# GetOverMassif/QSP-SLAM

Hardware: AMD Instinct MI355X
Metric: joint-opt iters/sec (BA+SDF) (higher is better)
Workload: dtype f32 as 2 x fp16 per operand (hi + 2^-11 lo'), 3 fp16 products per multiply-add, f32 accumulate (decoder); f64 (bundle adjustment)

## Files before the change

### include/qsp_hip.h

```cpp
#ifndef QSP_HIP_H
#define QSP_HIP_H

#include <stddef.h>
#include <stdint.h>

#ifdef __cplusplus
extern "C" {
#endif

enum {
    QSP_OK = 0,
    QSP_ERR_INVALID = 1,
    QSP_ERR_UNSUPPORTED = 2,
    QSP_ERR_DEVICE = 3,
    QSP_ERR_NO_DEVICE = 4
};

const char* qsp_last_error(void);
int qsp_version(void);
int qsp_device_count(void);


typedef struct {
    int32_t n_layers;
    int32_t code_len;
    int32_t latent_in_layer;
    const int32_t* in_dim;
    const int32_t* out_dim;
    const float* const* weight;
    const float* const* weight_g;
    const float* const* bias;
} qsp_decoder_desc;

typedef struct qsp_decoder qsp_decoder;

int qsp_decoder_create(const qsp_decoder_desc* desc, int device, qsp_decoder** out);
void qsp_decoder_destroy(qsp_decoder* dec);

enum { QSP_DEC_OPT_FORWARD_PRECISION = 1, QSP_DEC_OPT_JACOBIAN_PRECISION = 2, QSP_DEC_OPT_TILE_POINTS = 3,
       QSP_DEC_OPT_RENDER_SCREENING = 4, QSP_DEC_OPT_USE_TANH = 5, QSP_DEC_OPT_RANGE_FALLBACK = 6,
       QSP_DEC_OPT_SCREENING_MIN_SAMPLES = 7, QSP_DEC_OPT_NARROW_TILE = 8, QSP_DEC_OPT_SCREEN_AUDIT = 9,
       QSP_DEC_OPT_DEPTH_STAGING = 10 };
enum { QSP_DEC_CNT_RANGE_FALLBACKS = 1, QSP_DEC_CNT_ARENA_REUSED = 2, QSP_DEC_CNT_ARENA_CREATED = 3, QSP_DEC_CNT_NARROW_TILE = 4,
       QSP_DEC_CNT_SCREEN_FALLBACKS = 5 };
int64_t qsp_decoder_get_counter(qsp_decoder* dec, int32_t counter);
int qsp_decoder_set_option(qsp_decoder* dec, int32_t option, int32_t value);

int qsp_decode_sdf(qsp_decoder* dec, const float* code, const float* xyz, int64_t n, float* sdf_out);

int qsp_decode_sdf_screen(qsp_decoder* dec, const float* code, const float* xyz, int64_t n, float* s1_out);

int qsp_sdf_value_grad(qsp_decoder* dec, const float* code, const float* xyz, int64_t n, float* y, float* grad);

typedef struct {
    float k1, k2, k3, k4;
    float b1, b2;
    float lr;
    float s_damp;
    float cut_off;
    int32_t n_iter;
    int32_t n_depth;
    int32_t code_len;
} qsp_joint_cfg;

typedef struct qsp_refine_batch qsp_refine_batch;

int qsp_refine_batch_create(qsp_decoder* dec, const qsp_joint_cfg* cfg, int32_t n_obj,
                            const float* const* pts, const int32_t* n_pts,
                            const float* const* rays, const int32_t* n_rays,
                            const float* const* depth, const int32_t* n_fg,
                            int32_t n_hyp, const int32_t* hyp_obj, qsp_refine_batch** out);
void qsp_refine_batch_destroy(qsp_refine_batch* b);

int qsp_refine_batch_set_state(qsp_refine_batch* b, const float* t_cam_obj, const float* code);

// ... 518 lines not shown
```

### qsp_slam_amd/csrc/sdf_kernels.hpp

```cpp
#pragma once
#include <hip/hip_runtime.h>
#include <math.h>
#include <stdint.h>

#include "common.hpp"
#include "sdf_mlp.hpp"

namespace qsp {

constexpr int MAX_DEPTH = 64;
#ifndef QSP_NW_REND
#define QSP_NW_REND 16
#endif
#ifndef QSP_NW_SDF_MAX
#define QSP_NW_SDF_MAX 256
#endif
constexpr int NW_REND = QSP_NW_REND;
constexpr int NW_SDF_MAX = QSP_NW_SDF_MAX;
constexpr int NH = 71;
constexpr int PART_FLOATS = ((NJ * (NJ + 1) / 2 + 31) / 32) * 32;
__device__ __forceinline__ int tri72(int r, int c) { return r * NJ - (r * (r - 1)) / 2 + (c - r); }
__device__ __forceinline__ void part_store(float* __restrict__ slot, int ta, int tb, int lane, const f32x16& hacc) {
    const int r0 = 32 * ta + 4 * (lane >> 5), c = 32 * tb + (lane & 31);
    const int k = (NJ - 1) - r0, m = c < NJ ? c - r0 : -1;
// ... 565 lines not shown
        }
    }
    if (band_idx && screen_dmax && threadIdx.x < 64) {
#pragma unroll
        for (int o = 32; o > 0; o >>= 1) dmax = fmaxf(dmax, __shfl_xor(dmax, o, 64));
        if (threadIdx.x == 0 && dmax > 0.f) atomicMax(screen_dmax, __float_as_uint(dmax));
    }
    if (!(amax <= H2_MAX)) *P->range_flag = 1;
}

template <int NW, bool GRP = false>
__global__ __launch_bounds__(64 * NW) void k_mlp_fwd_h1(HypState* __restrict__ st, const ObjView* __restrict__ objs,
                                                            const float* __restrict__ rays, RefineCfg cfg, const MlpParams* __restrict__ P,
                                                            const int32_t* __restrict__ valid_rk, int64_t rk_stride,
                                                            float* __restrict__ sdf_valid, const int2* __restrict__ work,
                                                            int* __restrict__ qctl, const float* __restrict__ c0_all,
                                                            int32_t* __restrict__ band_idx, float band_th, int audit_one_in,
                                                            const int32_t* __restrict__ stage_idx) {
    extern __shared__ __attribute__((aligned(16))) unsigned char smem_raw[];
    MlpSmemH1& s = *reinterpret_cast<MlpSmemH1*>(smem_raw);
    __shared__ float Tsh[16];
    __shared__ int s_item;
    const int n_items = qctl[0];
    float amax = 0.f;
    int h_cached = -1;
    [[maybe_unused]] int dec_staged = -1;
    if constexpr (!GRP) {
        const MlpParams& Pp = *P;
        for (int i = threadIdx.x; i < HID; i += 64 * NW) s.w8[i] = Pp.w8[i];
#pragma unroll
        for (int l = 1; l < 8; ++l)
            for (int i = threadIdx.x; i < HID; i += 64 * NW) s.bias[(l - 1) * HID + i] = Pp.bias[l][i];
    }
    for (;;) {
        if (threadIdx.x == 0) s_item = atomicAdd(&qctl[1], 1);
        __syncthreads();
        const int item = s_item;
        if (item >= n_items) break;
        const int h = work[item].x, t = work[item].y;
        HypState& S = st[h];
        const int n = stage_idx ? S.n_stage : S.n_valid;
        const int32_t* stg = stage_idx ? stage_idx + h * rk_stride : nullptr;
        const ObjView ov = objs[S.obj];
        const float* R = rays + 3 * ov.ray_off;
        const int32_t* rk = valid_rk + h * rk_stride;
        float* out = sdf_valid + h * rk_stride;
        if (h != h_cached) {
            if (threadIdx.x >= 64 && threadIdx.x < 80) Tsh[threadIdx.x - 64] = S.T_oc[threadIdx.x - 64];
            for (int i = threadIdx.x; i < HID; i += 64 * NW) {
                s.c0[i] = c0_all[(size_t)h * 2 * HID + i];
                s.c4[i] = c0_all[(size_t)h * 2 * HID + HID + i];
            }
            h_cached = h;
        }
        if constexpr (GRP) {
            if (ov.dec != dec_staged) {
                const MlpParams& Pp = P[ov.dec];
                for (int i = threadIdx.x; i < HID; i += 64 * NW) s.w8[i] = Pp.w8[i];
#pragma unroll
                for (int l = 1; l < 8; ++l)
                    for (int i = threadIdx.x; i < HID; i += 64 * NW) s.bias[(l - 1) * HID + i] = Pp.bias[l][i];
                dec_staged = ov.dec;
            }
        }
        const float d_min = S.d_min, d_max = S.d_max;
        __syncthreads();
        if (threadIdx.x < H1_ROWS) {
            const int v = t * H1_ROWS + threadIdx.x;
            float x = 0, y = 0, z = 0;
            if (v < n) {
                const int e = rk[stg ? stg[v] : v];
                const int r = e >> 6, k = e & 63;
                const float d = depth_at(d_min, d_max, k, cfg.n_depth);
                xform(Tsh, R[3 * r] * d, R[3 * r + 1] * d, R[3 * r + 2] * d, x, y, z);
            }
            s.xin[4 * threadIdx.x + 0] = x;
            s.xin[4 * threadIdx.x + 1] = y;
            s.xin[4 * threadIdx.x + 2] = z;
            s.xin[4 * threadIdx.x + 3] = 0.f;
        }
        __syncthreads();
        if constexpr (GRP) mlp_tile_h1<2, NW>(s, P + ov.dec, amax);
        else mlp_tile_h1<2, NW>(s, P, amax);
        if (threadIdx.x < H1_ROWS) {
            int v = t * H1_ROWS + threadIdx.x;
            bool in = false, audit = false;
            if (v < n) {
                if (stg) v = stg[v];
                const float y = s.y[threadIdx.x];
                out[v] = y;
                in = !(fabsf(y) >= band_th);
                audit = !in && screen_audit_pick(h, v, cfg.iter, audit_one_in);
            }
            const unsigned long long m = __ballot(in || audit);
            const int lane = threadIdx.x & 63;
            int base = 0;
            if (lane == 0 && m) base = atomicAdd(&S.n_band, __popcll(m));
            base = __builtin_amdgcn_readfirstlane(base);
            if (in || audit) band_idx[h * rk_stride + base + __popcll(m & ((1ull << lane) - 1ull))] = audit ? (v | BAND_AUDIT_BIT) : v;
        }
    }
    if (!(amax <= H2_MAX)) *P->range_flag = 1;
}

struct RayScan {
    float d_u;
    int n_emit;
};

constexpr float SCAN_NONE = 1e30f;
constexpr int SCAN_RAYS = 512;
constexpr int SCAN_LD = MAX_DEPTH + 1;
__device__ __forceinline__ int scan_ray(float* row, int D, float d_min, float d_max, float th, float depth_obs, uint64_t& kept,
                                        float& res_out) {
    float occ[MAX_DEPTH];
    float Tl[MAX_DEPTH];
    uint64_t inband = 0;
    float acc = 1.f, d_u = 0.f;
#pragma unroll
    for (int k = 0; k < MAX_DEPTH; ++k) {
        if (k < D) {
            const float s = row[k];
            float o = 0.f;
            if (s < 0.5f * SCAN_NONE) {
                const float c = fminf(fmaxf(s, -th), th);
                o = 0.5f - c / (2.f * th);
                if (s > -th && s < th) inband |= 1ull << k;
            }
            occ[k] = o;
            const float d = depth_at(d_min, d_max, k, D);
            d_u += d * (o * acc);
            acc *= (1.f - o);
            Tl[k] = acc;
// ... 235 lines not shown
#pragma unroll 8
            for (int ks = 0; ks < TILE_P / 2; ++ks) hacc = mfma32t<!B3>(A[2 * ks * LDJ], B[2 * ks * LDJ], hacc);
            mfma_acc_settle<!B3>(hacc);
        }
        QSP_TSK(4)
    }
    if (wave < 6) part_store(partials + ((int64_t)h * nw_total + slot) * PART_FLOATS, ta, tb, lane, hacc);
    QSP_TSK(5)
    tsk_first = false;
  }
}

struct JtjArgs {
    const HypState* st;
    const ObjView* objs;
    const float* pts;
    const float* rays;
    RefineCfg cfg;
    const MlpParams* P;
    int nw_sdf, nw_total;
    const int32_t* rend_rk;
    const float* rend_deds;
    const float* rend_res;
    int64_t rk_stride;
    const uint8_t* pt_active;
    int64_t act_stride;
    float* res_out;
    float* rows_out;
    int64_t rows_stride;
    float* partials;
    const int2* work;
    int* qctl;
    const float* c0_all;
};
typedef const __attribute__((address_space(4))) JtjArgs* jtj_kargs_t;
__device__ __forceinline__ jtj_kargs_t jtj_kernargs() {
    auto p = __builtin_amdgcn_kernarg_segment_ptr();
    asm volatile("" : "+s"(p));
    return (jtj_kargs_t)p;
}

template <int NR, int NW = 4, bool NARROW = false, bool GRP = false>
__global__ __launch_bounds__(64 * NW) void k_mlp_jtj_h2(JtjArgs ) {
    constexpr int NT = 64 * NW;
    extern __shared__ __attribute__((aligned(16))) unsigned char smem_raw[];
    MlpSmem& s = *reinterpret_cast<MlpSmem*>(smem_raw);
    __shared__ float Tsh[16];
    __shared__ int s_item;
    constexpr int TP = 32 * NR, SUBS = NT / TP;
    [[maybe_unused]] bool staged = false;
    float amax = 0.f;
    int item = -1, t = 0;
    [[maybe_unused]] int dec = 0, dec_staged = -1;
    for (;;) {
        {
            const jtj_kargs_t A = jtj_kernargs();
            int tid = threadIdx.x;
            asm volatile("" : "+v"(tid));
            const bool fresh = item < 0;
            if (fresh) {
                if (tid == 0) s_item = atomicAdd(&A->qctl[3], 1);
                __syncthreads();
                item = __builtin_amdgcn_readfirstlane(s_item);
                if (item >= A->qctl[2]) break;
            } else {
                __syncthreads();
            }
            const int2 wk = A->work[item];
            const int h = wk.x, slot = wk.y;
            const HypState& S = A->st[h];
            const ObjView ov = A->objs[S.obj];
            const int nw_sdf = A->nw_sdf;
            const bool is_sdf = slot < nw_sdf;
            const int n = is_sdf ? ov.n_pts : S.n_render;
            if constexpr (GRP) dec = __builtin_amdgcn_readfirstlane(ov.dec);
            if (fresh) {
                t = is_sdf ? slot : slot - nw_sdf;
                if (tid < CODE_LEN) s.code[tid] = S.code[tid];
                if (tid >= 64 && tid < 80) Tsh[tid - 64] = S.T_oc[tid - 64];
                const float* c0 = A->c0_all + (size_t)h * 2 * HID;
                for (int i = tid; i < HID; i += NT) {
                    s.c0[i] = c0[i];
                    s.c4[i] = c0[HID + i];
                }
                __syncthreads();
            }
            if (tid < TP) {
                const int v = t * TP + tid;
                float x = 0, y = 0, z = 0, sc = 0.f, rr = 0.f;
                if (v < n) {
                    if (is_sdf) {
                        const float* Pc = A->pts + 3 * ov.pts_off;
                        const uint8_t* active = A->pt_active ? A->pt_active + h * A->act_stride : nullptr;
                        xform(Tsh, Pc[3 * v], Pc[3 * v + 1], Pc[3 * v + 2], x, y, z);
                        sc = (active && !active[v]) ? 0.f : 1.f;
                    } else {
                        const float* R = A->rays + 3 * ov.ray_off;
                        const int64_t ro = h * A->rk_stride;
                        const int e = A->rend_rk[ro + v];
                        const int r = e >> 6, k = e & 63;
                        const float d = depth_at(S.d_min, S.d_max, k, A->cfg.n_depth);
                        xform(Tsh, R[3 * r] * d, R[3 * r + 1] * d, R[3 * r + 2] * d, x, y, z);
                        sc = A->rend_deds[ro + v];
                        rr = A->rend_res[ro + v];
                    }
                }
                s.xin[4 * tid + 0] = x;
                s.xin[4 * tid + 1] = y;
                s.xin[4 * tid + 2] = z;
                s.xin[4 * tid + 3] = (v < n) ? 1.f : 0.f;
                s.rscale[tid] = sc;
                s.rres[tid] = rr;
            }
            __syncthreads();
        }
        {
            if constexpr (GRP) {
                const MlpParams* Pm = jtj_kernargs()->P + dec;
                mlp_tile_h2<true, 2, false, NR, NW, NARROW>(s, Pm, amax, dec != dec_staged);
                dec_staged = dec;
            } else {
                const MlpParams* Pm = jtj_kernargs()->P;
                mlp_tile_h2<true, 2, false, NR, NW, NARROW>(s, Pm, amax, !staged);
                staged = true;
            }
        }
        {
            asm volatile("" : "+s"(item), "+s"(t));
            const jtj_kargs_t A = jtj_kernargs();
            int tid = threadIdx.x;
            asm volatile("" : "+v"(tid));
            const int wave = __builtin_amdgcn_readfirstlane(tid >> 6), lane = tid & 63;
            const int2 wk = A->work[item];
            const int h = wk.x, slot = wk.y;
            const HypState& S = A->st[h];
            const ObjView ov = A->objs[S.obj];
            const int nw_sdf = A->nw_sdf, nw_total = A->nw_total;
            const bool is_sdf = slot < nw_sdf;
            const int n = is_sdf ? ov.n_pts : S.n_render;
            const int j0 = is_sdf ? slot : slot - nw_sdf;
            const int stride = is_sdf ? nw_sdf : nw_total - nw_sdf;
            const int pose_only = A->cfg.pose_only;
            const float hub = is_sdf ? A->cfg.b2 : A->cfg.b1;
            float* G = s.act;
            float* Jt = s.act + TILE_P * LDG;
            {
                const int p = tid / SUBS, sub = tid % SUBS;
                const float valid = s.xin[4 * p + 3];
                const float sc = s.rscale[p] * valid;
#pragma unroll
                for (int q = 0; q < CODE_LEN / SUBS; ++q) {
                    const int c = sub + SUBS * q;
                    Jt[p * LDJ + 7 + c] = pose_only ? 0.f : sc * G[p * LDG + c];
                }
                if (sub == 0) {
                    const float gx = sc * G[p * LDG + 64], gy = sc * G[p * LDG + 65], gz = sc * G[p * LDG + 66];
                    const float x = s.xin[4 * p], y = s.xin[4 * p + 1], z = s.xin[4 * p + 2];
                    Jt[p * LDJ + 0] = gx;
                    Jt[p * LDJ + 1] = gy;
                    Jt[p * LDJ + 2] = gz;
                    Jt[p * LDJ + 3] = gz * y - gy * z;
                    Jt[p * LDJ + 4] = gx * z - gz * x;
                    Jt[p * LDJ + 5] = gy * x - gx * y;
                    Jt[p * LDJ + 6] = pose_only ? 0.f : (gx * x + gy * y + gz * z);
                    float r = is_sdf ? s.y[p] : s.rres[p];
                    float w = pose_only ? 1.f : huber_w(r, hub);
                    if (is_sdf && s.rscale[p] == 0.f) w = 0.f;
                    Jt[p * LDJ + 71] = valid * (w * r);
                    float* res_out = A->res_out;
                    if (res_out && is_sdf && valid != 0.f) res_out[h * A->act_stride + t * TP + p] = r;
                }
                if (sub == 1) {
#pragma unroll
                    for (int c = NJ; c < LDJ; ++c) Jt[p * LDJ + c] = 0.f;
                }
            }
            __syncthreads();
            if (A->rows_out) {
                float* ro = A->rows_out + (int64_t)h * A->rows_stride * NJ + (int64_t)(is_sdf ? 0 : ov.n_pts) * NJ;
                for (int e = tid; e < TP * NJ; e += NT) {
                    const int p = e / NJ, c = e - p * NJ;
                    const int v = t * TP + p;
                    if (v < n) ro[(int64_t)v * NJ + c] = Jt[p * LDJ + c];
                }
            }
            float* out = A->partials + ((int64_t)h * nw_total + slot) * PART_FLOATS;
            const bool first = t == j0;
            if (NW == 4 || wave < 6) {
                const int ta0 = wave < 3 ? 0 : (wave < 5 ? 1 : 2), tb0 = wave < 3 ? wave : (wave < 5 ? wave - 2 : 2);
                f32x16 hacc;
                part_load(out, ta0, tb0, lane, first, hacc);
                const float* Aj = Jt + (lane >> 5) * LDJ + 32 * ta0 + (lane & 31);
                const float* Bj = Jt + (lane >> 5) * LDJ + 32 * tb0 + (lane & 31);
#pragma unroll 8
                for (int ks = 0; ks < TP / 2; ++ks) hacc = mfma32t<false>(Aj[2 * ks * LDJ], Bj[2 * ks * LDJ], hacc);
                part_store(out, ta0, tb0, lane, hacc);
            }
            if (NW == 4 && wave < 2) {
                const int ta1 = wave == 0 ? 1 : 2, tb1 = 2;
                f32x16 hacc;
                part_load(out, ta1, tb1, lane, first, hacc);
                const float* Aj = Jt + (lane >> 5) * LDJ + 32 * ta1 + (lane & 31);
                const float* Bj = Jt + (lane >> 5) * LDJ + 32 * tb1 + (lane & 31);
#pragma unroll 8
                for (int ks = 0; ks < TP / 2; ++ks) hacc = mfma32t<false>(Aj[2 * ks * LDJ], Bj[2 * ks * LDJ], hacc);
                part_store(out, ta1, tb1, lane, hacc);
            }
            t += stride;
            if (t * TP >= n) item = -1;
        }
    }
    if (!(amax <= H2_MAX)) *jtj_kernargs()->P->range_flag = 1;
}

__device__ __forceinline__ int tri_tile(int a, int b) {
    return a == 0 ? b : (a == 1 ? 2 + b : 5);
}

__device__ void exp_sim3_dev(const float* x, float* T) {
    const float v0 = x[0], v1 = x[1], v2 = x[2], w0 = x[3], w1 = x[4], w2 = x[5], sg = x[6];
    const float W[9] = {0.f, -w2, w1, w2, 0.f, -w0, -w1, w0, 0.f};
    float W2[9];
    for (int i = 0; i < 3; ++i)
        for (int j = 0; j < 3; ++j) W2[3 * i + j] = W[3 * i] * W[j] + W[3 * i + 1] * W[3 + j] + W[3 * i + 2] * W[6 + j];
    const float th = sqrtf(w0 * w0 + w1 * w1 + w2 * w2);
    const float es = expf(sg);
    float Rm[9], J[9];
    const float I[9] = {1, 0, 0, 0, 1, 0, 0, 0, 1};
    if (th <= 1e-8f) {
        const float c = (sg == 0.f) ? 1.f : (es - 1.f) / sg;
        for (int i = 0; i < 9; ++i) { Rm[i] = I[i]; J[i] = c * I[i]; }
    } else {
        const float sn = sinf(th), cs = cosf(th);
        const float a = es * sn, b = es * cs;
        const float c = (sg <= 1e-8f) ? 0.f : (es - 1.f) / sg;
        const float den = sg * sg + th * th;
        const float k1 = (a * sg + (1.f - b) * th) / den;
        const float k2 = c - ((b - 1.f) * sg + a * th) / den;
        for (int i = 0; i < 9; ++i) {
            Rm[i] = I[i] + W[i] * sn / th + W2[i] * (1.f - cs) / (th * th);
            J[i] = c * I[i] + k1 * W[i] / th + k2 * W2[i] / (th * th);
        }
// ... 534 lines not shown
```

### qsp_slam_amd/csrc/sdf_mlp.hpp

```cpp
#pragma once
#include <hip/hip_runtime.h>
#include <stdint.h>

namespace qsp {

typedef float f32x16 __attribute__((ext_vector_type(16)));

#ifndef QSP_EXP_VARIANT
#define QSP_EXP_VARIANT 0
#endif
#if (QSP_EXP_VARIANT & 16)
__device__ unsigned long long qsp_dbg_ts[96];
__device__ unsigned long long qsp_dbg_rt[96];
__device__ int qsp_dbg_n;
#define QSP_TS()                                                                        \
    if (blockIdx.x == 0 && blockIdx.y == 0 && threadIdx.x == 0 && ts_n < 96) {          \
        qsp_dbg_rt[ts_n] = __builtin_amdgcn_s_memrealtime();                            \
        qsp_dbg_ts[ts_n++] = __builtin_readcyclecounter();                              \
        qsp_dbg_n = ts_n;                                                               \
    }
#define QSP_TSK(i)                                                                      \
    if (blockIdx.x == 0 && threadIdx.x == 0 && tsk_first) {                             \
        qsp_dbg_rt[80 + (i)] = __builtin_amdgcn_s_memrealtime();                        \
        qsp_dbg_ts[80 + (i)] = __builtin_readcyclecounter();                            \
    }
#else
#define QSP_TS()
#define QSP_TSK(i)
#endif

constexpr int TILE_P = 64;
constexpr int HID = 512;
constexpr int CODE_LEN = 64;
constexpr int NIN = CODE_LEN + 3;
constexpr int SKIP_COL = HID - NIN;
constexpr int K4 = SKIP_COL + 3;
constexpr int KG4 = K4 / 8;
constexpr int K0_PAD = 96;
constexpr int LDA = HID + 4;
constexpr int LDST = 68;
constexpr int STASH_SHIFT = 1;
static_assert((SKIP_COL - STASH_SHIFT) % 4 == 0 && STASH_SHIFT + NIN <= LDST, "stash row: aligned quads of units 444.., 67 inputs");
constexpr int LDJ = 96;
constexpr int NJ = 72;
constexpr int MLP_THREADS = 512;
constexpr int HT_TILES = 6;

struct MlpParams {
    const float4* wf[8];
    const float4* wb[8];
    const float* bias[8];
    const float* w8;
    float b8;
    const float* w0c;
    const float* w4c;
    const float4* w0x;
    const float4* wf3[8];
    const float4* wb3[8];
    const float4* wfh[8];
    const float4* wbh[8];
    const float4* wbh4s;
// ... 1088 lines not shown
    if (NW == 8) return NR == 2 ? (wave & 1) : 0;
    return NR == 2 ? (wave < 2 ? r : wave - 2) : 0;
}
template <int PF, int NR, int NW, bool RT = false>
__device__ __forceinline__ void gemm_side_h2(const _Float16* __restrict__ img, const float4* __restrict__ wb, int wave, int lane,
                                             f32x4 (&out)[NR][4], int ks_run = HID / 16) {
    constexpr int KSH = HID / 16, CS = KSH * 2 * 64;
    const int c0 = side_c0<NR, NW>(wave);
    const float4* w0 = wb + (size_t)((c0 < 3 ? c0 : 0) * KSH * 2) * 64;
    WRingH<PF, 1> ring0;
    f32x16 g0[NR][1], g2[NR][1];
#pragma unroll
    for (int r = 0; r < NR; ++r)
#pragma unroll
        for (int i = 0; i < 16; ++i) { g0[r][0][i] = 0.f; g2[r][0][i] = 0.f; }
    if (side_count<NR, NW>(wave) == NR) {
        gemm_h2<KSH, PF, 1, NR, false, false, RT>(img, w0, CS, w0, CS, ring0, g0, g2, lane, ks_run);
    } else if (side_count<NR, NW>(wave) == 1) {
        f32x16 g01[1][1], g21[1][1];
#pragma unroll
        for (int i = 0; i < 16; ++i) { g01[0][0][i] = 0.f; g21[0][0][i] = 0.f; }
        gemm_h2<KSH, PF, 1, 1, false, false, RT>(img + side_row<NR, NW>(wave, 0) * 32 * LDH, w0, CS, w0, CS, ring0, g01, g21, lane, ks_run);
        g0[0][0] = g01[0][0];
        g2[0][0] = g21[0][0];
    }
#pragma unroll
    for (int r = 0; r < NR; ++r)
#pragma unroll
        for (int g = 0; g < 4; ++g)
#pragma unroll
            for (int q = 0; q < 4; ++q) out[r][g][q] = fmaf(g2[r][0][4 * g + q], 0.00048828125f, g0[r][0][4 * g + q]);
}

template <bool BWD, int PF, bool HAND = !BWD, int NR = 2, int NW = 4, bool NARROW = false>
__device__ __forceinline__ void mlp_tile_h2(MlpSmem& s, const MlpParams* __restrict__ Pm, float& amax, bool stage = true) {
    constexpr int NCB = 16 / NW, NT = 64 * NW;
    static_assert(!(BWD && HAND), "the forward+backward tile fetches each matrix's first slabs itself (layer 7 would hand over to the wrong one)");
    static_assert(!(NARROW && HAND), "the narrow form has no hand-over");
    int hts_n = 0;
    (void)hts_n;
    QSP_HTS()
    int tid = threadIdx.x;
    asm volatile("" : "+v"(tid));
    const int wave = __builtin_amdgcn_readfirstlane(tid >> 6);
    const int lane = tid & 63;
    const int h = lane >> 5;
    int oz;
    asm volatile("s_mov_b32 %0, 0" : "=s"(oz));
    const MlpParams& P = Pm[oz];
    constexpr int TP = 32 * NR;
    f32x16 acc[NR][NCB], acc2[NR][NCB];
    uint32_t mk[8][NR][NCB / 2];
    _Float16* img = reinterpret_cast<_Float16*>(s.act);
    float* bias_sh = s.stash;
    if (stage) {
        for (int i = tid; i < HID; i += NT) s.w8[i] = P.w8[i];
#pragma unroll
        for (int l = 1; l < 8; ++l)
            for (int i = tid; i < HID; i += NT) bias_sh[(l - 1) * HID + i] = P.bias[l][i];
    }
    if (tid < TP) {
        const f32x4 x = lds4(s.xin + 4 * tid);
        f16x8 hi, lo, z;
#pragma unroll
        for (int j = 0; j < 8; ++j) { hi[j] = (_Float16)0.f; lo[j] = (_Float16)0.f; z[j] = (_Float16)0.f; }
#pragma unroll
        for (int j = 0; j < 3; ++j) {
            hi[j] = (_Float16)x[j];
// ... 198 lines not shown
        if constexpr (NARROW) {
            f32x4 sk[NR][4];
            gemm_side_h2<PF, NR, NW, NARROW>(img, P.wbh4s, wave, lane, sk, NARROW ? (int)P.ks_out[4] : KSH);
            const int c0 = side_c0<NR, NW>(wave);
#pragma unroll
            for (int r = 0; r < NR; ++r) {
                if (r >= side_count<NR, NW>(wave)) break;
                const int p = 32 * side_row<NR, NW>(wave, r) + (lane & 31);
#pragma unroll
                for (int g = 0; g < 4; ++g) {
                    const int k0 = 32 * c0 + 8 * g + 4 * h;
#pragma unroll
                    for (int q = 0; q < 4; ++q)
                        if (k0 + q < NIN) s.stash[p * LDST + STASH_SHIFT + k0 + q] = sk[r][g][q];
                }
            }
        }
        QSP_BWDH(4, KSH, QSP_WBH(3))
        QSP_BWDH(3, KS4, QSP_WBH(2))
        QSP_BWDH(2, KSH, QSP_WBH(1))
        QSP_BWDH(1, KSH, QSP_WBH(1))
#undef QSP_BWDH
        {
            constexpr int BPT = HID / NT;
            float bnext[7 * BPT];
#pragma unroll
            for (int l = 1; l < 8; ++l)
#pragma unroll
                for (int i = 0; i < BPT; ++i) bnext[BPT * (l - 1) + i] = P.bias[l][tid + i * NT];
            __builtin_amdgcn_sched_barrier(0);
            f32x4 gl[NR][4];
            gemm_side_h2<PF, NR, NW, NARROW>(img, P.wbh[0], wave, lane, gl, NARROW ? (int)P.ks_out[0] : KSH);
            const int c0 = side_c0<NR, NW>(wave);
            __syncthreads();
#pragma unroll
            for (int r = 0; r < NR; ++r) {
                if (r >= side_count<NR, NW>(wave)) break;
                const int p = 32 * side_row<NR, NW>(wave, r) + (lane & 31);
#pragma unroll
                for (int g = 0; g < 4; ++g) {
                    const int k0 = 32 * c0 + 8 * g + 4 * h;
                    if (k0 < NIN) {
                        const float* st = s.stash + p * LDST + STASH_SHIFT + k0;
                        f32x4 v;
#pragma unroll
                        for (int q = 0; q < 4; ++q) v[q] = gl[r][g][q] + (k0 + q < NIN ? st[q] : 0.f);
                        *reinterpret_cast<f32x4*>(s.act + p * LDG + k0) = v;
                    }
                }
            }
            __syncthreads();
#pragma unroll
            for (int l = 1; l < 8; ++l)
#pragma unroll
                for (int i = 0; i < BPT; ++i) bias_sh[(l - 1) * HID + tid + i * NT] = bnext[BPT * (l - 1) + i];
        }
    }
#undef QSP_WH
#undef QSP_WBH
#undef QSP_PIN_ACC
}

constexpr int H1_ROWS = 128;
constexpr int LDH1 = HID + 8;
struct __attribute__((aligned(16))) MlpSmemH1 {
    _Float16 img[H1_ROWS * LDH1 + 64];
// ... 192 lines not shown
```

### qsp_slam_amd/csrc/sdf_refine.hip

```cpp
#include <hip/hip_runtime.h>
#include <math.h>
#include <stdint.h>
#include <stdio.h>
#include <stdlib.h>
#include <string.h>

#include <algorithm>
#include <limits>
#include <string>
#include <mutex>
#include <vector>

#include "../../include/qsp_hip.h"
#include "common.hpp"
#include "sdf_mlp.hpp"

#include "sdf_kernels.hpp"

#ifndef QSP_JTJ_WAVES_DEFAULT
#define QSP_JTJ_WAVES_DEFAULT 8
#endif
#ifndef QSP_SCREEN_WAVES_DEFAULT
#define QSP_SCREEN_WAVES_DEFAULT 4
#endif


using namespace qsp;

struct qsp_decoder {
    int device = 0;
    hipStream_t stream = nullptr;
    MlpParams P{};
    MlpParams* Pd = nullptr;
    std::vector<void*> allocs;
    double mac_per_point = 0;
    int code_len = CODE_LEN;
    int fwd_bf3 = 0;
    int jac_bf3 = 0;
    bool fp16_ok = true;
    int tile_p = 64;
    int* range_flag_h = nullptr;
    bool narrow_capable = false;
    float screen_margin = 0.f;
    int32_t depth_staging = 1;
    int32_t screen_audit = 100;
    int64_t screen_min_samples = -1;
    int range_fallback = 1;
    int64_t n_range_fallbacks = 0;
    int64_t n_screen_fallbacks = 0;
    std::recursive_mutex mu;
    struct qsp_refine_batch* arena = nullptr;
    int64_t n_arena_reuse = 0, n_arena_create = 0;
};

struct qsp_decoder_group {
    std::vector<qsp_decoder*> m;
    std::vector<qsp_decoder*> lock_order;
    int device = 0;
    MlpParams* Pd = nullptr;
    std::vector<MlpParams> Ph;
    struct qsp_refine_batch* arena = nullptr;
    int64_t n_arena_reuse = 0, n_arena_create = 0;
};

struct F32Override {
    qsp_decoder* d;
    int fwd, jac;
    explicit F32Override(qsp_decoder* d_) : d(d_), fwd(d_->fwd_bf3), jac(d_->jac_bf3) { d->fwd_bf3 = 0; d->jac_bf3 = 0; }
    ~F32Override() { d->fwd_bf3 = fwd; d->jac_bf3 = jac; }
};

static int embed_family(const qsp_decoder_desc* desc, const std::vector<std::vector<float>>& W,
                        std::vector<std::vector<float>>& Wc, std::vector<std::vector<float>>& Bc, std::vector<int>& src) {
    const int nl = desc->n_layers, m = nl - 1, L = desc->code_len;
    if (nl < 3 || nl > 9 || L < 1 || L > CODE_LEN)
        return qsp_fail(QSP_ERR_UNSUPPORTED, "decoder family: 2..8 hidden layers and a code of 1..64 are supported");
    int s = desc->latent_in_layer;
    const bool has_skip = s >= 0;
    if (!has_skip) {
        s = -1;
// ... 553 lines not shown
        case QSP_DEC_OPT_DEPTH_STAGING:
            if (value < 0 || value > 2) return qsp_fail(QSP_ERR_INVALID, "depth staging: 0 (off), 1 (large batches) or 2 (always)");
            d->depth_staging = (int32_t)value;
            return QSP_OK;
        case QSP_DEC_OPT_SCREEN_AUDIT:
            if (value < 0 || value > 1000000) return qsp_fail(QSP_ERR_INVALID, "screening audit: one in N out-of-band samples, N = 0 (off) .. 1e6");
            d->screen_audit = (int32_t)value;
            return QSP_OK;
        case QSP_DEC_OPT_SCREENING_MIN_SAMPLES:
            if (value < -1) return qsp_fail(QSP_ERR_INVALID, "screening threshold: -1 (automatic) or a sample count >= 0");
            d->screen_min_samples = value;
            return QSP_OK;
        case QSP_DEC_OPT_NARROW_TILE: {
            if (value != 0 && value != 1) return qsp_fail(QSP_ERR_INVALID, "narrow tile: 0 or 1");
            if (value && !d->narrow_capable) return qsp_fail(QSP_ERR_UNSUPPORTED, "narrow tile: this decoder fills most of the 8 x 512 shape");
            d->P.narrow = value;
            QSP_HIP(hipSetDevice(d->device));
            QSP_HIP(hipStreamSynchronize(d->stream));
            QSP_HIP(hipMemcpy(d->Pd, &d->P, sizeof(MlpParams), hipMemcpyHostToDevice));
            return QSP_OK;
        }
        case QSP_DEC_OPT_USE_TANH: {
            if (value != 0 && value != 1) return qsp_fail(QSP_ERR_INVALID, "use_tanh: 0 or 1");
            d->P.use_tanh = value;
            QSP_HIP(hipSetDevice(d->device));
            QSP_HIP(hipStreamSynchronize(d->stream));
            QSP_HIP(hipMemcpy(d->Pd, &d->P, sizeof(MlpParams), hipMemcpyHostToDevice));
            return QSP_OK;
        }
        case QSP_DEC_OPT_RANGE_FALLBACK:
            if (value != 0 && value != 1) return qsp_fail(QSP_ERR_INVALID, "range fallback: 0 or 1");
            d->range_fallback = value;
            return QSP_OK;
        default: return qsp_fail(QSP_ERR_INVALID, "qsp_decoder_set_option: unknown option");
    }
}

extern "C" int64_t qsp_decoder_get_counter(qsp_decoder* d, int32_t counter) {
    if (!d) return -1;
    switch (counter) {
        case QSP_DEC_CNT_RANGE_FALLBACKS: return d->n_range_fallbacks;
        case QSP_DEC_CNT_ARENA_REUSED: return d->n_arena_reuse;
        case QSP_DEC_CNT_ARENA_CREATED: return d->n_arena_create;
        case QSP_DEC_CNT_NARROW_TILE: return d->P.narrow ? 1 : 0;
        case QSP_DEC_CNT_SCREEN_FALLBACKS: return d->n_screen_fallbacks;
        default: return -1;
    }
}

static void batch_free(struct qsp_refine_batch* b);
extern "C" void qsp_decoder_destroy(qsp_decoder* d) {
    if (!d) return;
    (void)hipSetDevice(d->device);
    if (d->arena) batch_free(d->arena);
    d->arena = nullptr;
    for (void* p : d->allocs) (void)hipFree(p);
    if (d->range_flag_h) (void)hipHostFree(d->range_flag_h);
    if (d->stream) (void)hipStreamDestroy(d->stream);
    delete d;
}

template <class T> struct DevBuf {
    T* p = nullptr;
    DevBuf() = default;
    DevBuf(const DevBuf&) = delete;
    DevBuf& operator=(const DevBuf&) = delete;
// ... 167 lines not shown
static size_t align256(size_t n) { return (n + 255) & ~(size_t)255; }

struct CallLock {
    std::vector<std::unique_lock<std::recursive_mutex>> l;
    explicit CallLock(qsp_decoder* d) {
        if (d) l.emplace_back(d->mu);
    }
    explicit CallLock(qsp_decoder_group* g) {
        if (g)
            for (qsp_decoder* d : g->lock_order) l.emplace_back(d->mu);
    }
    explicit CallLock(qsp_refine_batch* b) {
        if (b && b->grp) *this = CallLock(b->grp);
        else if (b && b->dec) l.emplace_back(b->dec->mu);
    }
};

static int group_options(const qsp_decoder_group* g) {
    const qsp_decoder* a = g->m[0];
    for (size_t i = 1; i < g->m.size(); ++i) {
        const qsp_decoder* d = g->m[i];
        const char* what = nullptr;
        if (d->device != a->device) what = "device";
        else if (d->code_len != a->code_len) what = "code_len";
        else if (d->fwd_bf3 != a->fwd_bf3) what = "QSP_DEC_OPT_FORWARD_PRECISION";
        else if (d->jac_bf3 != a->jac_bf3) what = "QSP_DEC_OPT_JACOBIAN_PRECISION";
        else if (d->tile_p != a->tile_p) what = "QSP_DEC_OPT_TILE_POINTS";
        else if (d->P.narrow != a->P.narrow) what = "QSP_DEC_OPT_NARROW_TILE";
        else if (d->screen_margin != a->screen_margin) what = "QSP_DEC_OPT_RENDER_SCREENING";
        else if (d->screen_audit != a->screen_audit) what = "QSP_DEC_OPT_SCREEN_AUDIT";
        else if (d->screen_min_samples != a->screen_min_samples) what = "QSP_DEC_OPT_SCREENING_MIN_SAMPLES";
        else if (d->depth_staging != a->depth_staging) what = "QSP_DEC_OPT_DEPTH_STAGING";
        else if (d->range_fallback != a->range_fallback) what = "QSP_DEC_OPT_RANGE_FALLBACK";
        if (what) {
            const std::string msg = std::string("decoder group: member ") + std::to_string(i) + " differs from member 0 in " + what +
                                    " (the members of a group share it)";
            return qsp_fail(QSP_ERR_UNSUPPORTED, msg.c_str());
        }
    }
    return QSP_OK;
}
static int group_check(qsp_decoder_group* g) {
    const int rc = group_options(g);
    if (rc) return rc;
    bool stale = g->Ph.size() != g->m.size();
    g->Ph.resize(g->m.size());
    for (size_t i = 0; i < g->m.size(); ++i)
        if (memcmp(&g->Ph[i], &g->m[i]->P, sizeof(MlpParams)) != 0) {
            memcpy(&g->Ph[i], &g->m[i]->P, sizeof(MlpParams));
            stale = true;
        }
    if (stale) {
        QSP_HIP(hipSetDevice(g->device));
        QSP_HIP(hipStreamSynchronize(g->m[0]->stream));
        QSP_HIP(hipMemcpy(g->Pd, g->Ph.data(), sizeof(MlpParams) * g->m.size(), hipMemcpyHostToDevice));
    }
    return QSP_OK;
}

static int group_classes(const qsp_decoder_group* g, int32_t n_obj, const int32_t* cls) {
    if (!cls) return qsp_fail(QSP_ERR_INVALID, "decoder group: class index array is null");
    for (int o = 0; o < n_obj; ++o)
        if (cls[o] < 0 || cls[o] >= (int32_t)g->m.size())
            return qsp_fail(QSP_ERR_INVALID, "decoder group: class index out of range [0, number of members)");
    return QSP_OK;
}
// ... 305 lines not shown
                    const int32_t* stage_list = nullptr;
                    if (staged) {
                        const PlanTail pt_st{b->work_fwd, b->qctl, b->qctl + 4, nH, b->nw_sdf, nw_total - b->nw_sdf, H1_ROWS, 3};
                        hipLaunchKernelGGL(k_stage_list, dim3(nH), dim3(256), 0, s, b->st, b->objs, cfg, b->valid_rk, b->rk_stride, b->ray_voff,
                                           b->ray_stride, b->sdf_valid, b->ray_open, b->stage_idx, 0, sg == 0 ? 0 : k_mid,
                                           sg == 0 ? k_mid : cfg.n_depth, pt_st);
                        stage_list = b->stage_idx;
                    }
                    forward(screen_form(screen_waves(), grp), b->band_idx, cfg.cut_off + d->screen_margin, d->screen_audit, stage_list);
                    hipLaunchKernelGGL(k_plan, dim3(1), dim3(1024), 0, s, 2, b->st, b->objs, nH, b->nw_sdf, nw_total - b->nw_sdf,
                                       b->work_fwd, b->qctl, TILE_P);
                    forward(fwd_h2_form(false, grp), b->band_idx, (unsigned int*)(b->counters + 5));
                }
                screened_any = true;
            } else if (d->fwd_bf3 == 2)
                forward(fwd_h2_form(d->P.narrow, grp), nullptr, nullptr);
            else
                forward(fwd_form(d->fwd_bf3, grp));
            pm.end(1);
            pm.begin();
            const PlanTail pt_jtj{b->work_jtj, b->qctl, b->qctl + 5, nH, b->nw_sdf, nw_total - b->nw_sdf, cfg.tile_p, 1};
            launch(scan_kernel(), nH, s, b->st, b->objs, b->depth, cfg, b->valid_rk, b->rk_stride, b->ray_voff, b->ray_stride, b->sdf_valid,
                   b->rend_rk, b->rend_deds, b->rend_res, pt_jtj);
            pm.end(2);
        }
        pm.begin();
        if (cfg.pose_only)
            hipLaunchKernelGGL(k_plan, dim3(1), dim3(1024), 0, s, 1, b->st, b->objs, nH, b->nw_sdf, nw_total - b->nw_sdf,
                               b->work_jtj, b->qctl, cfg.tile_p);
        if (d->jac_bf3 == 2)
            launch(jtj_h2_form(d->P.narrow, cfg.tile_p, jtj_waves(), jtj_waves_t32(), grp), b->n_cu, s,
                   JtjArgs{b->st, b->objs, b->pts, b->rays, cfg, Pm, b->nw_sdf, nw_total, b->rend_rk, b->rend_deds, b->rend_res,
                           b->rk_stride, b->pt_active, b->act_stride, b->res_buf, b->rows, b->rows_stride, b->partials, b->work_jtj,
                           b->qctl, b->c0_all});
        else
            launch(jtj_form(d->jac_bf3, grp), b->n_cu, s, b->st, b->objs, b->pts, b->rays, cfg, Pm, b->nw_sdf, b->rend_rk, b->rend_deds,
                   b->rend_res, b->rk_stride, b->pt_active, b->act_stride, b->res_buf, b->rows, b->rows_stride, b->partials, nw_total,
                   b->work_jtj, b->qctl, b->c0_all);
        pm.end(0);
        pm.begin();
        hipLaunchKernelGGL(k_solve, dim3(nH), dim3(SOLVE_THREADS), 0, s, b->st, b->objs, cfg, b->partials, b->nw_sdf, nw_total,
                           b->pt_active, b->act_stride, b->trH, b->trb, b->trdx, b->counters, b->trrot);
        pm.end(2);
        if (cfg.pose_only && it == 4 && b->max_pts > 0)
            hipLaunchKernelGGL(k_inlier_filter, dim3((b->max_pts + 255) / 256, nH), dim3(256), 0, s, b->st, b->objs,
                               b->res_buf, b->act_stride, b->pt_active);
    }
    const hipEvent_t e_end = pm.mark();
    QSP_HIP(hipGetLastError());
    QSP_HIP(hipStreamSynchronize(s));
    if (range_hit(b->dec)) {
        *hit = true;
        return QSP_OK;
    }
    float dmax = 0.f;
    if (screened_any) {
        unsigned long long w[2] = {0, 0};
        QSP_HIP(hipMemcpy(w, b->counters + 5, sizeof(w), hipMemcpyDeviceToHost));
        const unsigned int bits = (unsigned int)w[0];
        memcpy(&dmax, &bits, sizeof(dmax));
        b->last_screen_dmax = dmax;
        b->last_audit_wrong = (int32_t)(w[0] >> 32);
        b->last_audited = (int64_t)w[1];
        if (!(dmax <= SCREEN_TRUST * b->dec->screen_margin) || b->last_audit_wrong > 0) {
            *screen_hit = true;
            return QSP_OK;
        }
// ... 373 lines not shown
                                             const float* const* depth, const int32_t* n_fg, const int32_t* obj_class, int32_t n_hyp,
                                             const int32_t* hyp_obj, const float* t_cam_obj, const float* code,
                                             float* t_cam_obj_out, float* code_out, float* loss_out, uint8_t* is_good_out) {
    if (!g) return qsp_fail(QSP_ERR_INVALID, "qsp_reconstruct_objects_group: null group");
    const CallLock lk(g);
    int rc = group_check(g);
    if (!rc && n_obj > 0) rc = group_classes(g, n_obj, obj_class);
    if (rc) return rc;
    return reconstruct_objects(g->m[0], g, obj_class, cfg, n_obj, pts, n_pts, rays, n_rays, depth, n_fg, n_hyp, hyp_obj, t_cam_obj,
                               code, t_cam_obj_out, code_out, loss_out, is_good_out);
}

extern "C" int qsp_estimate_pose_group(qsp_decoder_group* g, int32_t n, const float* t_co_se3, const float* scale,
                                       const float* const* pts, const int32_t* n_pts, const float* code, const int32_t* obj_class,
                                       int32_t n_iter, float* t_co_out) {
    if (!g) return qsp_fail(QSP_ERR_INVALID, "qsp_estimate_pose_group: null group");
    const CallLock lk(g);
    int rc = group_check(g);
    if (!rc && n > 0) rc = group_classes(g, n, obj_class);
    if (rc) return rc;
    return estimate_pose(g->m[0], g, obj_class, n, t_co_se3, scale, pts, n_pts, code, n_iter, t_co_out);
}

#if (QSP_EXP_VARIANT & 16)
extern "C" int qsp_debug_timestamps(unsigned long long* out , int* n, unsigned long long* rt ) {
    (void)hipDeviceSynchronize();
    (void)hipMemcpyFromSymbol(out, HIP_SYMBOL(qsp::qsp_dbg_ts), sizeof(unsigned long long) * 96);
    if (rt) (void)hipMemcpyFromSymbol(rt, HIP_SYMBOL(qsp::qsp_dbg_rt), sizeof(unsigned long long) * 96);
    (void)hipMemcpyFromSymbol(n, HIP_SYMBOL(qsp::qsp_dbg_n), sizeof(int));
    return 0;
}
#endif

#if QSP_PHASE_CLOCK
extern "C" int qsp_debug_phase_ticks(unsigned long long* out ) {
    (void)hipDeviceSynchronize();
    (void)hipMemcpyFromSymbol(out, HIP_SYMBOL(qsp::qsp_phase_ticks), sizeof(unsigned long long) * 48);
    static const unsigned long long zero[48] = {};
    (void)hipMemcpyToSymbol(HIP_SYMBOL(qsp::qsp_phase_ticks), zero, sizeof(zero));
    return 0;
}
#endif

#include "mesh_extract.hpp"
#include "detections.hpp"
```

### qsp_slam_amd/decoder.py

```python
import ctypes as C
import ast
import json
import os

import numpy as np

from . import _lib


class DeepSdfDecoder(object):

    def __init__(self, layers, latent_in=(4,), code_len=64, device=0):
        L = _lib.lib()
        latent_in = tuple(latent_in or ())
        if len(latent_in) > 1:
            raise _lib.QspError(_lib.QSP_ERR_UNSUPPORTED, "at most one latent_in layer is supported")
        n = len(layers)
        self._keep = []
        in_dim = np.array([l[0].shape[1] for l in layers], np.int32)
        out_dim = np.array([l[0].shape[0] for l in layers], np.int32)
        w = [_lib.f32c(l[0]) for l in layers]
        g = [None if l[1] is None else _lib.f32c(np.asarray(l[1]).reshape(-1)) for l in layers]
        b = [_lib.f32c(l[2]) for l in layers]
        fpp = _lib.c_float_p * n
# ... 31 lines not shown
        if name != "fp16x2":
            self.render_screening = 0.0

    def set_forward_precision(self, mode):
        _lib.check(_lib.lib().qsp_decoder_set_option(self.handle, 1, int(mode)))

    def set_jacobian_precision(self, mode):
        _lib.check(_lib.lib().qsp_decoder_set_option(self.handle, 2, int(mode)))

    def set_tile_points(self, n):
        _lib.check(_lib.lib().qsp_decoder_set_option(self.handle, 3, int(n)))
        self.tile_points = int(n)

    def set_screening_min_samples(self, n=-1):
        _lib.check(_lib.lib().qsp_decoder_set_option(self.handle, 7, int(n)))

    def set_depth_staging(self, on=True):
        _lib.check(_lib.lib().qsp_decoder_set_option(self.handle, 10, 2 if on == "always" else (1 if on else 0)))

    def set_screen_audit(self, one_in=100):
        _lib.check(_lib.lib().qsp_decoder_set_option(self.handle, 9, int(one_in)))

    def set_render_screening(self, margin=0.01):
        _lib.check(_lib.lib().qsp_decoder_set_option(self.handle, 4, int(round(1e6 * float(margin or 0.0)))))
        self.render_screening = float(margin or 0.0)

    def set_use_tanh(self, on):
        _lib.check(_lib.lib().qsp_decoder_set_option(self.handle, 5, 1 if on else 0))
        self.use_tanh = bool(on)

    def set_range_fallback(self, on):
        _lib.check(_lib.lib().qsp_decoder_set_option(self.handle, 6, 1 if on else 0))

    @property
    def range_fallbacks(self):
        return int(_lib.lib().qsp_decoder_get_counter(self.handle, 1))

    @property
    def screen_fallbacks(self):
        return int(_lib.lib().qsp_decoder_get_counter(self.handle, 5))

    @property
    def narrow_tile(self):
        return bool(_lib.lib().qsp_decoder_get_counter(self.handle, 4))

    def set_narrow_tile(self, on):
        _lib.check(_lib.lib().qsp_decoder_set_option(self.handle, 8, 1 if on else 0))

    @property
    def arena_stats(self):
        L = _lib.lib()
        return int(L.qsp_decoder_get_counter(self.handle, 2)), int(L.qsp_decoder_get_counter(self.handle, 3))

    def decode_sdf_screen(self, code, x):
        x = _lib.f32c(x)
        code = _lib.f32c(np.asarray(code)[: self.code_len])
        out = np.empty(x.shape[0], np.float32)
        _lib.check(_lib.lib().qsp_decode_sdf_screen(self.handle, _lib.fptr(code), _lib.fptr(x), x.shape[0], _lib.fptr(out)))
        return out

    def close(self):
        if getattr(self, "handle", None):
            _lib.lib().qsp_decoder_destroy(self.handle)
            self.handle = None

    def __del__(self):
# ... 113 lines not shown
```

Baseline: 5833.

## Prefetch next JtJ work item's inputs during MLP tile in idle wave

Result: no change. 5853, median of 6 (+0.3%).

```diff
diff --git a/include/qsp_hip.h b/include/qsp_hip.h
--- a/include/qsp_hip.h
+++ b/include/qsp_hip.h
@@ -40,7 +40,7 @@
 enum { QSP_DEC_OPT_FORWARD_PRECISION = 1, QSP_DEC_OPT_JACOBIAN_PRECISION = 2, QSP_DEC_OPT_TILE_POINTS = 3,
        QSP_DEC_OPT_RENDER_SCREENING = 4, QSP_DEC_OPT_USE_TANH = 5, QSP_DEC_OPT_RANGE_FALLBACK = 6,
        QSP_DEC_OPT_SCREENING_MIN_SAMPLES = 7, QSP_DEC_OPT_NARROW_TILE = 8, QSP_DEC_OPT_SCREEN_AUDIT = 9,
-       QSP_DEC_OPT_DEPTH_STAGING = 10 };
+       QSP_DEC_OPT_DEPTH_STAGING = 10, QSP_DEC_OPT_ITEM_PREFETCH = 11 };
 enum { QSP_DEC_CNT_RANGE_FALLBACKS = 1, QSP_DEC_CNT_ARENA_REUSED = 2, QSP_DEC_CNT_ARENA_CREATED = 3, QSP_DEC_CNT_NARROW_TILE = 4,
        QSP_DEC_CNT_SCREEN_FALLBACKS = 5 };
 int64_t qsp_decoder_get_counter(qsp_decoder* dec, int32_t counter);
diff --git a/qsp_slam_amd/csrc/sdf_kernels.hpp b/qsp_slam_amd/csrc/sdf_kernels.hpp
--- a/qsp_slam_amd/csrc/sdf_kernels.hpp
+++ b/qsp_slam_amd/csrc/sdf_kernels.hpp
@@ -621,11 +621,14 @@
         for (int l = 1; l < 8; ++l)
             for (int i = threadIdx.x; i < HID; i += 64 * NW) s.bias[(l - 1) * HID + i] = Pp.bias[l][i];
     }
+    QSP_TSI_INIT()
     for (;;) {
+        QSP_TSI(1, 0)
         if (threadIdx.x == 0) s_item = atomicAdd(&qctl[1], 1);
         __syncthreads();
         const int item = s_item;
         if (item >= n_items) break;
+        QSP_TSI(1, 1)
         const int h = work[item].x, t = work[item].y;
         HypState& S = st[h];
         const int n = stage_idx ? S.n_stage : S.n_valid;
@@ -669,8 +672,10 @@
             s.xin[4 * threadIdx.x + 3] = 0.f;
         }
         __syncthreads();
+        QSP_TSI(1, 2)
         if constexpr (GRP) mlp_tile_h1<2, NW>(s, P + ov.dec, amax);
         else mlp_tile_h1<2, NW>(s, P, amax);
+        QSP_TSI(1, 3)
         if (threadIdx.x < H1_ROWS) {
             int v = t * H1_ROWS + threadIdx.x;
             bool in = false, audit = false;
@@ -688,6 +693,7 @@
             base = __builtin_amdgcn_readfirstlane(base);
             if (in || audit) band_idx[h * rk_stride + base + __popcll(m & ((1ull << lane) - 1ull))] = audit ? (v | BAND_AUDIT_BIT) : v;
         }
+        QSP_TSI(1, 4)
     }
     if (!(amax <= H2_MAX)) *P->range_flag = 1;
 }
@@ -989,6 +995,7 @@
     const int2* work;
     int* qctl;
     const float* c0_all;
+    int32_t item_prefetch;
 };
 typedef const __attribute__((address_space(4))) JtjArgs* jtj_kargs_t;
 __device__ __forceinline__ jtj_kargs_t jtj_kernargs() {
@@ -996,6 +1003,99 @@
     asm volatile("" : "+s"(p));
     return (jtj_kargs_t)p;
 }
+
+__device__ __forceinline__ void jtj_stage_row(jtj_kargs_t A, const float* T, int h, const HypState& S, const ObjView& ov, bool is_sdf,
+                                              int n, int v, int row, float* xin, float* rscale, float* rres) {
+    float x = 0, y = 0, z = 0, sc = 0.f, rr = 0.f;
+    if (v < n) {
+        if (is_sdf) {
+            const float* Pc = A->pts + 3 * ov.pts_off;
+            const uint8_t* active = A->pt_active ? A->pt_active + h * A->act_stride : nullptr;
+            xform(T, Pc[3 * v], Pc[3 * v + 1], Pc[3 * v + 2], x, y, z);
+            sc = (active && !active[v]) ? 0.f : 1.f;
+        } else {
+            const float* R = A->rays + 3 * ov.ray_off;
+            const int64_t ro = h * A->rk_stride;
+            const int e = A->rend_rk[ro + v];
+            const int r = e >> 6, k = e & 63;
+            const float d = depth_at(S.d_min, S.d_max, k, A->cfg.n_depth);
+            xform(T, R[3 * r] * d, R[3 * r + 1] * d, R[3 * r + 2] * d, x, y, z);
+            sc = A->rend_deds[ro + v];
+            rr = A->rend_res[ro + v];
+        }
+    }
+    xin[4 * row + 0] = x;
+    xin[4 * row + 1] = y;
+    xin[4 * row + 2] = z;
+    xin[4 * row + 3] = (v < n) ? 1.f : 0.f;
+    rscale[row] = sc;
+    rres[row] = rr;
+}
+
+struct __attribute__((aligned(16))) JtjNext {
+    float xin[TILE_P * 4], rscale[TILE_P], rres[TILE_P];
+    int state, item, t, dec;
+};
+static_assert(sizeof(MlpSmem) + sizeof(JtjNext) + 16 * sizeof(float) + sizeof(int) <= 160 * 1024,
+              "MlpSmem + the item loop's static LDS (Tsh, s_item, JtjNext) must fit the 160 KB of a workgroup");
+struct JtjNoPrefetch {
+    MlpSmem& s;
+    JtjNext& nx;
+    int item, t;
+    __device__ __forceinline__ void operator()(int) const {}
+};
+template <int NR, bool GRP>
+struct JtjPrefetch {
+    MlpSmem& s;
+    JtjNext& nx;
+    int item, t;
+    __device__ __forceinline__ void operator()(int lane) const {
+        constexpr int TP = 32 * NR;
+        const jtj_kargs_t A = jtj_kernargs();
+        if (!A->item_prefetch) return;
+        int vz = 0;
+        asm volatile("" : "+v"(lane), "+v"(vz));
+        const int nw_sdf = A->nw_sdf, nw_total = A->nw_total;
+        int it = item, h, slot, n, t2;
+        bool is_sdf;
+        const HypState* S;
+        ObjView ov;
+        const auto look = [&]() {
+            const int2 wk = A->work[it + vz];
+            h = wk.x, slot = wk.y;
+            S = &A->st[h];
+            ov = A->objs[S->obj];
+            is_sdf = slot < nw_sdf;
+            n = is_sdf ? ov.n_pts : S->n_render;
+        };
+        look();
+        t2 = t + (is_sdf ? nw_sdf : nw_total - nw_sdf);
+        if (__builtin_amdgcn_readfirstlane(t2 * TP >= n)) {
+            int popped = 0;
+            if (lane == 0) popped = atomicAdd(&A->qctl[3], 1);
+            it = __builtin_amdgcn_readfirstlane(popped);
+            if (it >= A->qctl[2]) {
+                if (lane == 0) nx.state = 2;
+                return;
+            }
+            look();
+            t2 = is_sdf ? slot : slot - nw_sdf;
+            s.code[lane] = S->code[lane];
+            const float* c0 = A->c0_all + (size_t)h * 2 * HID;
+            for (int i = lane; i < HID; i += 64) {
+                s.c0[i] = c0[i];
+                s.c4[i] = c0[HID + i];
+            }
+        }
+        if (lane < TP) jtj_stage_row(A, S->T_oc, h, *S, ov, is_sdf, n, t2 * TP + lane, lane, nx.xin, nx.rscale, nx.rres);
+        if (lane == 0) {
+            nx.item = it;
+            nx.t = t2;
+            nx.dec = GRP ? ov.dec : 0;
+            nx.state = 1;
+        }
+    }
+};
 
 template <int NR, int NW = 4, bool NARROW = false, bool GRP = false>
 __global__ __launch_bounds__(64 * NW) void k_mlp_jtj_h2(JtjArgs ) {
@@ -1009,8 +1109,33 @@
     float amax = 0.f;
     int item = -1, t = 0;
     [[maybe_unused]] int dec = 0, dec_staged = -1;
+    constexpr bool PRE = NR == 1 || (NW == 8 && !GRP);
+    __shared__ JtjNext nx;
+    if constexpr (PRE) {
+        if (threadIdx.x == 0) nx.state = 0;
+        __syncthreads();
+    }
+    QSP_TSI_INIT()
     for (;;) {
-        {
+        QSP_TSI(0, 0)
+        const int pre = PRE ? __builtin_amdgcn_readfirstlane(nx.state) : 0;
+        if (pre == 2) break;
+        if (pre == 1) {
+            int tid = threadIdx.x;
+            asm volatile("" : "+v"(tid));
+            __syncthreads();
+            item = __builtin_amdgcn_readfirstlane(nx.item);
+            t = __builtin_amdgcn_readfirstlane(nx.t);
+            if constexpr (GRP) dec = __builtin_amdgcn_readfirstlane(nx.dec);
+            QSP_TSI(0, 1)
+            if (tid < TP) {
+                *reinterpret_cast<f32x4*>(s.xin + 4 * tid) = lds4(nx.xin + 4 * tid);
+                s.rscale[tid] = nx.rscale[tid];
+                s.rres[tid] = nx.rres[tid];
+            }
+            __syncthreads();
+            QSP_TSI(0, 2)
+        } else {
             const jtj_kargs_t A = jtj_kernargs();
             int tid = threadIdx.x;
             asm volatile("" : "+v"(tid));
@@ -1023,6 +1148,7 @@
             } else {
                 __syncthreads();
             }
+            QSP_TSI(0, 1)
             const int2 wk = A->work[item];
             const int h = wk.x, slot = wk.y;
             const HypState& S = A->st[h];
@@ -1042,46 +1168,23 @@
                 }
                 __syncthreads();
             }
-            if (tid < TP) {
-                const int v = t * TP + tid;
-                float x = 0, y = 0, z = 0, sc = 0.f, rr = 0.f;
-                if (v < n) {
-                    if (is_sdf) {
-                        const float* Pc = A->pts + 3 * ov.pts_off;
-                        const uint8_t* active = A->pt_active ? A->pt_active + h * A->act_stride : nullptr;
-                        xform(Tsh, Pc[3 * v], Pc[3 * v + 1], Pc[3 * v + 2], x, y, z);
-                        sc = (active && !active[v]) ? 0.f : 1.f;
-                    } else {
-                        const float* R = A->rays + 3 * ov.ray_off;
-                        const int64_t ro = h * A->rk_stride;
-                        const int e = A->rend_rk[ro + v];
-                        const int r = e >> 6, k = e & 63;
-                        const float d = depth_at(S.d_min, S.d_max, k, A->cfg.n_depth);
-                        xform(Tsh, R[3 * r] * d, R[3 * r + 1] * d, R[3 * r + 2] * d, x, y, z);
-                        sc = A->rend_deds[ro + v];
-                        rr = A->rend_res[ro + v];
-                    }
-                }
-                s.xin[4 * tid + 0] = x;
-                s.xin[4 * tid + 1] = y;
-                s.xin[4 * tid + 2] = z;
-                s.xin[4 * tid + 3] = (v < n) ? 1.f : 0.f;
-                s.rscale[tid] = sc;
-                s.rres[tid] = rr;
-            }
+            if (tid < TP) jtj_stage_row(A, Tsh, h, S, ov, is_sdf, n, t * TP + tid, tid, s.xin, s.rscale, s.rres);
             __syncthreads();
+            QSP_TSI(0, 2)
         }
         {
+            const std::conditional_t<PRE, JtjPrefetch<NR, GRP>, JtjNoPrefetch> next{s, nx, item, t};
             if constexpr (GRP) {
                 const MlpParams* Pm = jtj_kernargs()->P + dec;
-                mlp_tile_h2<true, 2, false, NR, NW, NARROW>(s, Pm, amax, dec != dec_staged);
+                mlp_tile_h2<true, 2, false, NR, NW, NARROW>(s, Pm, amax, dec != dec_staged, next);
                 dec_staged = dec;
             } else {
                 const MlpParams* Pm = jtj_kernargs()->P;
-                mlp_tile_h2<true, 2, false, NR, NW, NARROW>(s, Pm, amax, !staged);
+                mlp_tile_h2<true, 2, false, NR, NW, NARROW>(s, Pm, amax, !staged, next);
                 staged = true;
             }
         }
+        QSP_TSI(0, 3)
         {
             asm volatile("" : "+s"(item), "+s"(t));
             const jtj_kargs_t A = jtj_kernargs();
@@ -1133,6 +1236,7 @@
                 }
             }
             __syncthreads();
+            QSP_TSI(0, 4)
             if (A->rows_out) {
                 float* ro = A->rows_out + (int64_t)h * A->rows_stride * NJ + (int64_t)(is_sdf ? 0 : ov.n_pts) * NJ;
                 for (int e = tid; e < TP * NJ; e += NT) {
@@ -1165,6 +1269,7 @@
             }
             t += stride;
             if (t * TP >= n) item = -1;
+            QSP_TSI(0, 5)
         }
     }
     if (!(amax <= H2_MAX)) *jtj_kernargs()->P->range_flag = 1;
diff --git a/qsp_slam_amd/csrc/sdf_mlp.hpp b/qsp_slam_amd/csrc/sdf_mlp.hpp
--- a/qsp_slam_amd/csrc/sdf_mlp.hpp
+++ b/qsp_slam_amd/csrc/sdf_mlp.hpp
@@ -24,9 +24,20 @@
         qsp_dbg_rt[80 + (i)] = __builtin_amdgcn_s_memrealtime();                        \
         qsp_dbg_ts[80 + (i)] = __builtin_readcyclecounter();                            \
     }
+__device__ unsigned long long qsp_item_ticks[2][8];
+#define QSP_TSI_INIT() unsigned long long tsi_last = __builtin_amdgcn_s_memrealtime();
+#define QSP_TSI(kern, i)                                                                \
+    if (threadIdx.x == 0) {                                                             \
+        const unsigned long long now_ = __builtin_amdgcn_s_memrealtime();               \
+        atomicAdd(&qsp_item_ticks[kern][i], now_ - tsi_last);                           \
+        if ((i) == 0) atomicAdd(&qsp_item_ticks[kern][7], 1ull);                        \
+        tsi_last = now_;                                                                \
+    }
 #else
 #define QSP_TS()
 #define QSP_TSK(i)
+#define QSP_TSI_INIT()
+#define QSP_TSI(kern, i)
 #endif
 
 constexpr int TILE_P = 64;
@@ -1181,8 +1192,10 @@
             for (int q = 0; q < 4; ++q) out[r][g][q] = fmaf(g2[r][0][4 * g + q], 0.00048828125f, g0[r][0][4 * g + q]);
 }
 
-template <bool BWD, int PF, bool HAND = !BWD, int NR = 2, int NW = 4, bool NARROW = false>
-__device__ __forceinline__ void mlp_tile_h2(MlpSmem& s, const MlpParams* __restrict__ Pm, float& amax, bool stage = true) {
+struct NoNext { __device__ __forceinline__ void operator()(int) const {} };
+template <bool BWD, int PF, bool HAND = !BWD, int NR = 2, int NW = 4, bool NARROW = false, class NEXT = NoNext>
+__device__ __forceinline__ void mlp_tile_h2(MlpSmem& s, const MlpParams* __restrict__ Pm, float& amax, bool stage = true,
+                                            const NEXT& next = NEXT()) {
     constexpr int NCB = 16 / NW, NT = 64 * NW;
     static_assert(!(BWD && HAND), "the forward+backward tile fetches each matrix's first slabs itself (layer 7 would hand over to the wrong one)");
     static_assert(!(NARROW && HAND), "the narrow form has no hand-over");
@@ -1447,6 +1460,7 @@
             f32x4 gl[NR][4];
             gemm_side_h2<PF, NR, NW, NARROW>(img, P.wbh[0], wave, lane, gl, NARROW ? (int)P.ks_out[0] : KSH);
             const int c0 = side_c0<NR, NW>(wave);
+            if (wave == NW - 1) next(lane);
             __syncthreads();
 #pragma unroll
             for (int r = 0; r < NR; ++r) {
diff --git a/qsp_slam_amd/csrc/sdf_refine.hip b/qsp_slam_amd/csrc/sdf_refine.hip
--- a/qsp_slam_amd/csrc/sdf_refine.hip
+++ b/qsp_slam_amd/csrc/sdf_refine.hip
@@ -46,6 +46,7 @@
     int32_t screen_audit = 100;
     int64_t screen_min_samples = -1;
     int range_fallback = 1;
+    int32_t item_prefetch = 1;
     int64_t n_range_fallbacks = 0;
     int64_t n_screen_fallbacks = 0;
     std::recursive_mutex mu;
@@ -665,6 +666,10 @@
             if (value != 0 && value != 1) return qsp_fail(QSP_ERR_INVALID, "range fallback: 0 or 1");
             d->range_fallback = value;
             return QSP_OK;
+        case QSP_DEC_OPT_ITEM_PREFETCH:
+            if (value != 0 && value != 1) return qsp_fail(QSP_ERR_INVALID, "item prefetch: 0 or 1");
+            d->item_prefetch = value;
+            return QSP_OK;
         default: return qsp_fail(QSP_ERR_INVALID, "qsp_decoder_set_option: unknown option");
     }
 }
@@ -898,6 +903,7 @@
         else if (d->screen_min_samples != a->screen_min_samples) what = "QSP_DEC_OPT_SCREENING_MIN_SAMPLES";
         else if (d->depth_staging != a->depth_staging) what = "QSP_DEC_OPT_DEPTH_STAGING";
         else if (d->range_fallback != a->range_fallback) what = "QSP_DEC_OPT_RANGE_FALLBACK";
+        else if (d->item_prefetch != a->item_prefetch) what = "QSP_DEC_OPT_ITEM_PREFETCH";
         if (what) {
             const std::string msg = std::string("decoder group: member ") + std::to_string(i) + " differs from member 0 in " + what +
                                     " (the members of a group share it)";
@@ -1269,7 +1275,7 @@
             launch(jtj_h2_form(d->P.narrow, cfg.tile_p, jtj_waves(), jtj_waves_t32(), grp), b->n_cu, s,
                    JtjArgs{b->st, b->objs, b->pts, b->rays, cfg, Pm, b->nw_sdf, nw_total, b->rend_rk, b->rend_deds, b->rend_res,
                            b->rk_stride, b->pt_active, b->act_stride, b->res_buf, b->rows, b->rows_stride, b->partials, b->work_jtj,
-                           b->qctl, b->c0_all});
+                           b->qctl, b->c0_all, d->item_prefetch});
         else
             launch(jtj_form(d->jac_bf3, grp), b->n_cu, s, b->st, b->objs, b->pts, b->rays, cfg, Pm, b->nw_sdf, b->rend_rk, b->rend_deds,
                    b->rend_res, b->rk_stride, b->pt_active, b->act_stride, b->res_buf, b->rows, b->rows_stride, b->partials, nw_total,
@@ -1709,6 +1715,16 @@
 }
 #endif
 
+#if (QSP_EXP_VARIANT & 16)
+extern "C" int qsp_debug_item_ticks(unsigned long long* out ) {
+    (void)hipDeviceSynchronize();
+    (void)hipMemcpyFromSymbol(out, HIP_SYMBOL(qsp::qsp_item_ticks), sizeof(unsigned long long) * 16);
+    static const unsigned long long zero[16] = {};
+    (void)hipMemcpyToSymbol(HIP_SYMBOL(qsp::qsp_item_ticks), zero, sizeof(zero));
+    return 0;
+}
+#endif
+
 #if QSP_PHASE_CLOCK
 extern "C" int qsp_debug_phase_ticks(unsigned long long* out ) {
     (void)hipDeviceSynchronize();
diff --git a/qsp_slam_amd/decoder.py b/qsp_slam_amd/decoder.py
--- a/qsp_slam_amd/decoder.py
+++ b/qsp_slam_amd/decoder.py
@@ -87,6 +87,9 @@
     def set_range_fallback(self, on):
         _lib.check(_lib.lib().qsp_decoder_set_option(self.handle, 6, 1 if on else 0))
 
+    def set_item_prefetch(self, on=True):
+        _lib.check(_lib.lib().qsp_decoder_set_option(self.handle, 11, 1 if on else 0))
+
     @property
     def range_fallbacks(self):
         return int(_lib.lib().qsp_decoder_get_counter(self.handle, 1))
```
